# ShunyaoWang/quadruped_locomotion

Measured on NVIDIA B200. Metric: contact-force QPs solved/sec, higher is better.
Workload: dtype f64

## Files before the change

quadruped_locomotion_b200/csrc/qlb_api.cu:

```cuda
#include <cuda_runtime.h>
#include <dlfcn.h>
#include <nccl.h>

#include <cmath>
#include <cstdio>
#include <cstdlib>
#include <cstring>
#include <mutex>
#include <new>

#include "qlb.h"
#include "qlb_aux.cuh"
#include "qlb_gen.cuh"
#include "qlb_qp_dense.cuh"
#include "qlb_records.cuh"
#include "qlb_solve.cuh"
#include "qlb_solve_quad.cuh"
#include "qlb_solve_fused.cuh"
#include "qlb_solve_single.cuh"
#include "qlb_swing.cuh"
#include "qlb_tick.cuh"

using namespace qlb;

#ifndef QLB_PIPE
#define QLB_PIPE 3
#endif
constexpr int kPipe = QLB_PIPE;

struct qlb_context {
  int device = 0;
  int sm_count = 0;
  int blocks_per_sm_quad[2] = {0, 0};
  int blocks_per_sm_first[2] = {0, 0};
  qlb_params params;
  qlb_leg_model legs[QLB_NUM_LEGS];
  DeviceModel* d_model = nullptr;
  DeviceParams* d_params = nullptr;
  DeviceLimbDynamics* d_limb = nullptr;
  DeviceLimbDynamicsT<float>* d_limb_f = nullptr;
  bool have_limb = false;
  DeviceModelT<float>* d_model_f = nullptr;
  DeviceParamsT<float>* d_params_f = nullptr;
  int blocks_per_sm_quad_f[2] = {0, 0};
  int blocks_per_sm_first_f[2] = {0, 0};
  int blocks_per_sm_quad_m[2] = {0, 0};
  int blocks_per_sm_first_m[2] = {0, 0};
  int pipeline = QLB_PIPELINE_FUSED;
  int blocks_per_sm_single[2][2][2] = {};
  std::recursive_mutex mu;
  int fused_bps_cap = 0;
  bool use_tma = true;
  bool f32_pure = false;
  unsigned long long* d_counter = nullptr;
  unsigned* d_list[8] = {};
  size_t list_cap[8] = {};
  uint64_t solve_calls = 0;
  cudaEvent_t slot_done[8] = {};
  int last_slot = 0;
  double* d_stats = nullptr;
  cudaStream_t stream = nullptr;
  cudaStream_t pipe[kPipe] = {};
  double* d_in = nullptr;
  double* d_out = nullptr;
  uint8_t* d_mask = nullptr;
  uint32_t* d_flags = nullptr;
  unsigned char* d_prev = nullptr;
  size_t prev_cap = 0;
  unsigned char* d_qp = nullptr;
  size_t qp_bytes = 0;
  unsigned char* d_rec = nullptr;
  size_t rec_cap = 0;
  size_t cap = 0;
  uint64_t launches = 0;
  char last_error[256] = {0};
};

namespace {

constexpr int kHostInRows = 12 + 7 + 6 + 7 + 6 + 4 + 12;
constexpr int kHostOutRows = 12 + 12 + 6 + 6;
#ifndef QLB_CHUNK_LOG2
#define QLB_CHUNK_LOG2 17
#endif
constexpr size_t kChunk = size_t(1) << QLB_CHUNK_LOG2;

struct DeviceGuard {
  int prev = -1;
  explicit DeviceGuard(int dev) {
// ... 195 lines not shown
}

bool make_mask_map(CUtensorMap* m, const uint8_t* ptr, unsigned long long B, int cols) {
  EncodeTiledFn fn = encode_tiled_fn();
  if (!fn) return false;
  const cuuint64_t gdim[1] = {(cuuint64_t)B};
  const cuuint64_t gstride[1] = {0};
  const cuuint32_t box[1] = {(cuuint32_t)cols};
  const cuuint32_t estr[1] = {1u};
  return fn(m, CU_TENSOR_MAP_DATA_TYPE_UINT8, 1, const_cast<uint8_t*>(ptr), gdim, gstride, box, estr, CU_TENSOR_MAP_INTERLEAVE_NONE,
            CU_TENSOR_MAP_SWIZZLE_NONE, CU_TENSOR_MAP_L2_PROMOTION_NONE, CU_TENSOR_MAP_FLOAT_OOB_FILL_NONE) == CUDA_SUCCESS;
}

template <typename T, typename C, int MODE>
int launch_single(qlb_context* ctx, SolveArgsT<T>& a, cudaStream_t st, const int bps_ipm) {
  using SG = Staging<T, MODE, QLB_SUPER>;
  using FL = FusedLayout<T, C, MODE, QLB_SUPER>;
  const T* src[SG::kNumSeg];
  for (int s = 0; s < SG::kNumSeg; s++) src[s] = SG::source(a, s);
  bool tma = ctx->use_tma && a.B >= 64 && a.B < 0x7fffff00ull && ((a.B * sizeof(T)) % 16 == 0);
  for (int s = 0; s < SG::kNumSeg && tma; s++)
    if (src[s] && !aligned16(src[s])) tma = false;
  FusedMaps maps;
  std::memset(&maps, 0, sizeof maps);
  for (int s = 0; s < SG::kNumSeg && tma; s++)
    if (src[s] && !make_map<T>(&maps.seg[s], src[s], a.B, SG::rows(s))) tma = false;
  if (tma && (SG::kCols < 16 || !aligned16(a.mask) || !make_mask_map(&maps.mask, a.mask, a.B, SG::kCols))) tma = false;
  const unsigned long long ntiles = (a.B + 7) / 8;
  const unsigned long long want = (ntiles + kFusedWarps - 1) / kFusedWarps;
  int bps = ctx->blocks_per_sm_single[sizeof(T) == 4 ? 1 : 0][MODE][tma ? 1 : 0];
  if (ctx->fused_bps_cap > 0 && bps > ctx->fused_bps_cap) bps = ctx->fused_bps_cap;
  const unsigned long long cap = (unsigned long long)ctx->sm_count * bps;
  const unsigned grid = (unsigned)(want < cap ? want : cap);
  if (tma) qlb_single_kernel<T, C, MODE, QLB_SUPER, true><<<grid, kFusedThreads, FL::kTotal, st>>>(a, maps);
  else qlb_single_kernel<T, C, MODE, QLB_SUPER, false><<<grid, kFusedThreads, FL::kTotal, st>>>(a, maps);
  QLB_CUDA(ctx, cudaGetLastError());
  ctx->launches++;
  const unsigned long long capq = (unsigned long long)ctx->sm_count * bps_ipm;
  const unsigned long long wantq = (ntiles + 3) / 4;
  qlb_quad_kernel<T, C, MODE, 2><<<(unsigned)(wantq < capq ? wantq : capq), kQuadThreads, 0, st>>>(a);
  QLB_CUDA(ctx, cudaGetLastError());
  ctx->launches++;
  QLB_CUDA(ctx, cudaEventRecord(ctx->slot_done[ctx->last_slot], st));
  return QLB_OK;
}

template <typename T, typename C, int MODE>
bool prepare_single_kernels(qlb_context* ctx) {
  using FL = FusedLayout<T, C, MODE, QLB_SUPER>;
  int* out = ctx->blocks_per_sm_single[sizeof(T) == 4 ? 1 : 0][MODE];
  if (cudaFuncSetAttribute(qlb_single_kernel<T, C, MODE, QLB_SUPER, false>, cudaFuncAttributeMaxDynamicSharedMemorySize, FL::kTotal) != cudaSuccess ||
      cudaFuncSetAttribute(qlb_single_kernel<T, C, MODE, QLB_SUPER, true>, cudaFuncAttributeMaxDynamicSharedMemorySize, FL::kTotal) != cudaSuccess ||
      cudaFuncSetAttribute(qlb_single_kernel<T, C, MODE, QLB_SUPER, false>, cudaFuncAttributePreferredSharedMemoryCarveout, cudaSharedmemCarveoutMaxShared) != cudaSuccess ||
      cudaFuncSetAttribute(qlb_single_kernel<T, C, MODE, QLB_SUPER, true>, cudaFuncAttributePreferredSharedMemoryCarveout, cudaSharedmemCarveoutMaxShared) != cudaSuccess)
    return false;
  if (cudaOccupancyMaxActiveBlocksPerMultiprocessor(&out[0], qlb_single_kernel<T, C, MODE, QLB_SUPER, false>, kFusedThreads, FL::kTotal) != cudaSuccess ||
      cudaOccupancyMaxActiveBlocksPerMultiprocessor(&out[1], qlb_single_kernel<T, C, MODE, QLB_SUPER, true>, kFusedThreads, FL::kTotal) != cudaSuccess)
    return false;
  return out[0] >= 1 && out[1] >= 1;
}

template <int MODE>
int launch_solve(qlb_context* ctx, SolveArgs& a, cudaStream_t st) {
  const int rc = prepare_slot(ctx, a, st);
  if (rc != QLB_OK) return rc;
  if (ctx->pipeline == QLB_PIPELINE_FUSED) return launch_single<double, double, MODE>(ctx, a, st, ctx->blocks_per_sm_quad[MODE]);
// ... 263 lines not shown
      cudaOccupancyMaxActiveBlocksPerMultiprocessor(&ctx->blocks_per_sm_first_f[0], qlb_quad_first_kernel<float, float, 0>, kQuadThreads, 0) != cudaSuccess ||
      cudaOccupancyMaxActiveBlocksPerMultiprocessor(&ctx->blocks_per_sm_first_f[1], qlb_quad_first_kernel<float, float, 1>, kQuadThreads, 0) != cudaSuccess)
    return fail(QLB_ERR_CUDA);
  if (cudaOccupancyMaxActiveBlocksPerMultiprocessor(&ctx->blocks_per_sm_quad_m[0], qlb_quad_kernel<float, double, 0, 2>, kQuadThreads, 0) != cudaSuccess ||
      cudaOccupancyMaxActiveBlocksPerMultiprocessor(&ctx->blocks_per_sm_quad_m[1], qlb_quad_kernel<float, double, 1, 2>, kQuadThreads, 0) != cudaSuccess ||
      cudaOccupancyMaxActiveBlocksPerMultiprocessor(&ctx->blocks_per_sm_first_m[0], qlb_quad_first_kernel<float, double, 0>, kQuadThreads, 0) != cudaSuccess ||
      cudaOccupancyMaxActiveBlocksPerMultiprocessor(&ctx->blocks_per_sm_first_m[1], qlb_quad_first_kernel<float, double, 1>, kQuadThreads, 0) != cudaSuccess)
    return fail(QLB_ERR_CUDA);
  if (!prepare_single_kernels<double, double, 0>(ctx) || !prepare_single_kernels<double, double, 1>(ctx) ||
      !prepare_single_kernels<float, double, 0>(ctx) || !prepare_single_kernels<float, double, 1>(ctx)) {
    cudaGetLastError();
    return fail(QLB_ERR_CUDA);
  }
  if (const char* e = std::getenv("QLB_FUSED_BPS")) ctx->fused_bps_cap = std::atoi(e);
  if (const char* e = std::getenv("QLB_PIPELINE")) {
    if (!std::strcmp(e, "three_pass")) ctx->pipeline = QLB_PIPELINE_THREE_PASS;

    if (!std::strcmp(e, "fused_notma")) ctx->use_tma = false;
  }
  if (max_batch > 0 && ensure_capacity(ctx, max_batch) != QLB_OK) return fail(QLB_ERR_ALLOC);
  *out = ctx;
  return QLB_OK;
}

int qlb_destroy(qlb_context* ctx) {
  if (!ctx) return QLB_OK;
  DeviceGuard guard(ctx->device);
  if (ctx->stream) { cudaStreamSynchronize(ctx->stream); cudaStreamDestroy(ctx->stream); }
  for (int i = 0; i < kPipe; i++)
    if (ctx->pipe[i]) { cudaStreamSynchronize(ctx->pipe[i]); cudaStreamDestroy(ctx->pipe[i]); }
  cudaFree(ctx->d_model); cudaFree(ctx->d_params); cudaFree(ctx->d_counter); cudaFree(ctx->d_stats);
  cudaFree(ctx->d_model_f); cudaFree(ctx->d_params_f); cudaFree(ctx->d_limb); cudaFree(ctx->d_limb_f);
  cudaFree(ctx->d_in); cudaFree(ctx->d_out); cudaFree(ctx->d_mask); cudaFree(ctx->d_flags); cudaFree(ctx->d_rec); cudaFree(ctx->d_qp); cudaFree(ctx->d_prev);
  for (int i = 0; i < 8; i++) cudaFree(ctx->d_list[i]);
  for (int i = 0; i < 8; i++)
    if (ctx->slot_done[i]) cudaEventDestroy(ctx->slot_done[i]);
  cudaGetLastError();
  delete ctx;
  return QLB_OK;
}

int qlb_set_params(qlb_context* ctx, const qlb_params* params) {
  QLB_GUARD(ctx);
  if (!ctx || !params) return QLB_ERR_INVALID_ARGUMENT;
  if (!params_ok(params)) return QLB_ERR_INVALID_ARGUMENT;
  DeviceGuard guard(ctx->device);
  DeviceParams hp;
  build_device_params(params, &hp);
  QLB_CUDA(ctx, cudaDeviceSynchronize());
  QLB_CUDA(ctx, cudaMemcpy(ctx->d_params, &hp, sizeof hp, cudaMemcpyHostToDevice));
  DeviceParamsT<float> hpf;
  narrow_params(hp, &hpf);
  QLB_CUDA(ctx, cudaMemcpy(ctx->d_params_f, &hpf, sizeof hpf, cudaMemcpyHostToDevice));
  ctx->params = *params;
  return QLB_OK;
}

int qlb_get_params(const qlb_context* ctx, qlb_params* params) {
  if (!ctx || !params) return QLB_ERR_INVALID_ARGUMENT;
  *params = ctx->params;
  return QLB_OK;
}

int qlb_set_f32_core(qlb_context* ctx, int core) {
  QLB_GUARD(ctx);
  if (!ctx) return QLB_ERR_NOT_INITIALISED;
  if (core != QLB_F32_CORE_FP32 && core != QLB_F32_CORE_FP64) return QLB_ERR_INVALID_ARGUMENT;
// ... 1031 lines not shown
```

quadruped_locomotion_b200/csrc/qlb_solve.cuh:

```cuda
#pragma once

#include "qlb_device.cuh"

namespace qlb {

constexpr int kModePolish = 0, kModeIpm = 1, kModeDone = 2;
constexpr int kPolishPasses = 10;
constexpr double kNeighbourhood = 1e-3;

template <typename T>
struct SolveArgsT {
  unsigned long long B;
  const T* q;
  const T* quat;
  const T* wrench;
  const uint8_t* mask;
  const T* mu;
  const T* normals;
  const T* pose;
  const T* twist;
  const T* tpose;
  const T* ttwist;
  T* grf;
  T* tau;
  uint32_t* flags;
  T* netwrench;
  T* wrench_out;
  unsigned long long* counter;
  unsigned long long* counter2;
  unsigned* list;
  unsigned* list_pat;
  unsigned* list_count;
  unsigned long long* counter3;
  unsigned* list2;
  unsigned* list2_count;
  const DeviceModelT<T>* model;
  const DeviceParamsT<T>* params;
  const DeviceParamsT<double>* params64;
};
using SolveArgs = SolveArgsT<double>;

template <typename T>
__device__ __forceinline__ void quat_rel_log(const T* qt, const T* q, T (&v)[3]) {
  const T aw = qt[0], ax = -qt[1], ay = -qt[2], az = -qt[3];
  T w = aw * q[0] - ax * q[1] - ay * q[2] - az * q[3];
  T x = aw * q[1] + ax * q[0] + ay * q[3] - az * q[2];
  T y = aw * q[2] - ax * q[3] + ay * q[0] + az * q[1];
  T z = aw * q[3] + ax * q[2] - ay * q[1] + az * q[0];
  if (w < T(0.0)) { w = -w; x = -x; y = -y; z = -z; }
  const T n = sqrt(x * x + y * y + z * z);
  T k = T(2.0);
  if (n >= T(1e-12)) k = T(2.0) * atan2(n, w) / n;
  v[0] = k * x; v[1] = k * y; v[2] = k * z;
}

}
```

quadruped_locomotion_b200/csrc/qlb_solve_fused.cuh:

```cuda
#pragma once

#include <cuda.h>

#include "qlb_solve_quad.cuh"

namespace qlb {

#ifndef QLB_SUPER
#define QLB_SUPER 2
#endif
#ifndef QLB_DBAS_MAX_ROUNDS
#define QLB_DBAS_MAX_ROUNDS 40
#endif

template <typename real, int MODE, int SUPER>
struct Staging {
  static constexpr int kCols = 8 * SUPER;
  static constexpr int kRow = kCols * (int)sizeof(real);
  __host__ __device__ static constexpr int align(int x) { return (x + 127) & ~127; }
  static constexpr int kNumSeg = (MODE == 1) ? 7 : 5;
  __host__ __device__ static constexpr int rows(int s) {
    return (MODE == 1) ? (s == 0 ? 12 : s == 1 ? 7 : s == 2 ? 6 : s == 3 ? 7 : s == 4 ? 6 : s == 5 ? 4 : 12)
                       : (s == 0 ? 12 : s == 1 ? 4 : s == 2 ? 6 : s == 3 ? 4 : 12);
  }
// ... 31 lines not shown
  asm volatile(
      "{\n"
      ".reg .pred p;\n"
      "mbarrier.try_wait.parity.shared::cta.b64 p, [%1], %2;\n"
      "selp.u32 %0, 1, 0, p;\n"
      "}\n" : "=r"(ok) : "r"(bar), "r"(parity) : "memory");
  return ok != 0u;
}
__device__ __forceinline__ void mbar_wait(uint32_t bar, uint32_t parity) {
  for (unsigned spins = 0; spins < (1u << 24); spins++) {
    const bool ok = mbar_try_wait(bar, parity);
    if (__all_sync(kFull, ok)) break;
  }
}
__device__ __forceinline__ void tma_load_2d(uint32_t dst, const CUtensorMap* map, int c0, int c1, uint32_t bar) {
  asm volatile("cp.async.bulk.tensor.2d.shared::cluster.global.mbarrier::complete_tx::bytes [%0], [%1, {%2, %3}], [%4];"
               ::"r"(dst), "l"(map), "r"(c0), "r"(c1), "r"(bar) : "memory");
}
__device__ __forceinline__ void tma_load_1d(uint32_t dst, const CUtensorMap* map, int c0, uint32_t bar) {
  asm volatile("cp.async.bulk.tensor.1d.shared::cluster.global.mbarrier::complete_tx::bytes [%0], [%1, {%2}], [%3];"
               ::"r"(dst), "l"(map), "r"(c0), "r"(bar) : "memory");
}
__device__ __forceinline__ void cp_async_4(uint32_t dst, const void* src, int valid) {
  asm volatile("cp.async.ca.shared.global [%0], [%1], 4, %2;" ::"r"(dst), "l"(src), "r"(valid) : "memory");
}
__device__ __forceinline__ void cp_async_elem(uint32_t dst, const double* src) {
  asm volatile("cp.async.ca.shared.global [%0], [%1], 8;" ::"r"(dst), "l"(src) : "memory");
}
__device__ __forceinline__ void cp_async_elem(uint32_t dst, const float* src) {
  asm volatile("cp.async.ca.shared.global [%0], [%1], 4;" ::"r"(dst), "l"(src) : "memory");
}
__device__ __forceinline__ void cp_async_commit() { asm volatile("cp.async.commit_group;" ::: "memory"); }
__device__ __forceinline__ void cp_async_wait_all() { asm volatile("cp.async.wait_group 0;" ::: "memory"); }

__device__ __forceinline__ int nth_set_bit(unsigned m, const int j) {
#pragma unroll
  for (int i = 0; i < 7; i++)
    if (i < j) m &= m - 1u;
  return m ? (__ffs(m) - 1) : -1;
}

template <typename real, int MODE, int SUPER, bool TMA>
__device__ __forceinline__ void stage_issue(const SolveArgsT<real>& a, const FusedMaps& maps, const unsigned long long box,
                                            unsigned char* stage, const uint32_t bar, const int lane) {
  using SG = Staging<real, MODE, SUPER>;
  const real* src[SG::kNumSeg];
#pragma unroll
  for (int s = 0; s < SG::kNumSeg; s++) src[s] = SG::source(a, s);
  if (TMA) {
    if (lane == 0) {
      uint32_t bytes = 0;
#pragma unroll
      for (int s = 0; s < SG::kNumSeg; s++)
        if (src[s] != nullptr) bytes += SG::rows(s) * SG::kRow;
      bytes += SG::kCols;
      mbar_expect_tx(bar, bytes);
      const uint32_t dst = smem_u32(stage);
#pragma unroll
      for (int s = 0; s < SG::kNumSeg; s++)
        if (src[s] != nullptr) tma_load_2d(dst + SG::offset(s), &maps.seg[s], (int)(box * (unsigned long long)SG::kCols), 0, bar);
      tma_load_1d(dst + SG::kMaskOff, &maps.mask, (int)(box * (unsigned long long)SG::kCols), bar);
    }
  } else {
    const unsigned long long B = a.B;
    constexpr int kRowsPerPass = 32 / SG::kCols;
    const int col = lane % SG::kCols;
    unsigned long long bx = box * (unsigned long long)SG::kCols + col;
    if (bx >= B) bx = B - 1;
#pragma unroll
    for (int s = 0; s < SG::kNumSeg; s++) {
      if (src[s] == nullptr) continue;
      const uint32_t dst = smem_u32(stage) + SG::offset(s);
#pragma unroll
// ... 195 lines not shown
```

quadruped_locomotion_b200/csrc/qlb_solve_single.cuh:

```cuda
#pragma once

#include "qlb_solve_fused.cuh"

namespace qlb {

#ifndef QLB_FUSED_MIN_CTAS
#define QLB_FUSED_MIN_CTAS 1
#endif
#ifndef QLB_FUSED_MIN_CTAS_F32
#define QLB_FUSED_MIN_CTAS_F32 1
#endif
#ifndef QLB_FUSED_THREADS
#define QLB_FUSED_THREADS 384
#endif
#ifndef QLB_DYNAMIC_PART
#define QLB_DYNAMIC_PART 4
#endif
#ifndef QLB_STASH_CAP
#define QLB_STASH_CAP 22
#endif
#ifndef QLB_ROUND_LOW
#define QLB_ROUND_LOW 8
#endif
constexpr int kFusedThreads = QLB_FUSED_THREADS;
constexpr int kFusedWarps = kFusedThreads / 32;
template <typename real> constexpr int fused_min_ctas() { return sizeof(real) == 4 ? QLB_FUSED_MIN_CTAS_F32 : QLB_FUSED_MIN_CTAS; }
template <typename real> constexpr int fused_smem_budget() { return (228 / fused_min_ctas<real>() - 1) * 1024; }

constexpr int kStashLane = 16;
constexpr int kSlFoot = 6, kSlMu = 9, kSlY = 10, kSlU = 13;
template <typename real, typename creal, int CAP>
struct StashLayout {
  static constexpr int kQ = 4 * CAP;
  static constexpr int kLaneBytes = kStashLane * kQ * (int)sizeof(creal);
  static constexpr int kJBytes = 12 * kQ * (int)sizeof(real);
  static constexpr int kBBytes = 6 * CAP * (int)sizeof(creal);
  static constexpr int kHBytes = 4 * CAP * 4;
  static constexpr int kBytes = ((kLaneBytes + kJBytes + kBBytes + kHBytes) + 15) & ~15;
};

template <typename real, typename creal, int MODE, int SUPER>
struct FusedLayout {
  static constexpr int kCtlWords = 8;
  static constexpr int kBarBytes = (kFusedWarps * 8 + 63) & ~63;
  static constexpr int kFixed = ((((int)sizeof(DeviceParamsT<real>) + 15) & ~15) + (((int)sizeof(CoreConst<creal>) + 15) & ~15) + kBarBytes +
                                 kFusedWarps * kCtlWords * 4 + 127) & ~127;
  static constexpr int kStatic = (int)sizeof(DeviceModelT<double>) + 128;
  static constexpr int kStage = Staging<real, MODE, SUPER>::kBytes;
  static constexpr int stash_bytes(int c) {
    return ((kStashLane * 4 * c * (int)sizeof(creal) + 12 * 4 * c * (int)sizeof(real) + 6 * c * (int)sizeof(creal) + 16 * c) + 15) & ~15;
  }
  static constexpr int warp_bytes(int c) { return (kStage + stash_bytes(c) + 127) & ~127; }
  static constexpr int cap_for(int c) { return (kStatic + kFixed + kFusedWarps * warp_bytes(c) <= fused_smem_budget<real>() || c <= 8) ? c : cap_for(c - 1); }
  static constexpr int kCap = cap_for(QLB_STASH_CAP);
  static_assert(kCap >= 10, "stash too small");
  static_assert(stash_bytes(kCap) == StashLayout<real, creal, kCap>::kBytes, "layout mismatch");
  static constexpr int kWarpBytes = warp_bytes(kCap);
  static constexpr int kTotal = kFixed + kFusedWarps * kWarpBytes;
  static_assert(kStatic + kTotal <= fused_smem_budget<real>(), "shared memory budget");
};

template <typename real, typename creal, int CAP>
struct WarpStash {
  creal* sl;
  real* sj;
  creal* sb;
  uint32_t* sh;
  __device__ WarpStash(unsigned char* base) {
    using SL = StashLayout<real, creal, CAP>;
    sl = reinterpret_cast<creal*>(base);
    sj = reinterpret_cast<real*>(base + SL::kLaneBytes);
    sb = reinterpret_cast<creal*>(base + SL::kLaneBytes + SL::kJBytes);
    sh = reinterpret_cast<uint32_t*>(base + SL::kLaneBytes + SL::kJBytes + SL::kBBytes);
  }
};


template <typename real, typename creal, int CAP>
__device__ __forceinline__ void stash_load(const WarpStash<real, creal, CAP>& ws, const int slot, const int leg, RoundState<creal>& q) {
  constexpr int Q = 4 * CAP;
  const int e = 4 * slot + leg;
  const uint32_t w1 = ws.sh[CAP + slot];
  q.idx = ws.sh[slot];
  q.gscale = __uint_as_float(ws.sh[2 * CAP + slot]);
  q.mask = w1 & 0xFu;
  q.alive = (w1 >> leg) & 1u;
  q.rounds = (int)(w1 >> 24);
  const unsigned pat = (w1 >> (4 + 5 * leg)) & 31u;
  q.a0 = (int)(pat & 1u);
  q.sg1 = ((pat >> 1) & 3u) == 1u ? -1 : (((pat >> 1) & 3u) == 2u ? 1 : 0);
  q.sg2 = ((pat >> 3) & 3u) == 1u ? -1 : (((pat >> 3) & 3u) == 2u ? 1 : 0);
  creal foot[3];
#pragma unroll
  for (int c = 0; c < 3; c++) {
    q.At[0][c] = ws.sl[c * Q + e];
    q.At[1][c] = ws.sl[(3 + c) * Q + e];
    foot[c] = ws.sl[(kSlFoot + c) * Q + e];
  }
  {
    creal t2[3];
    t2[0] = q.At[0][1] * q.At[1][2] - q.At[0][2] * q.At[1][1];
    t2[1] = q.At[0][2] * q.At[1][0] - q.At[0][0] * q.At[1][2];
    t2[2] = q.At[0][0] * q.At[1][1] - q.At[0][1] * q.At[1][0];
    const creal rn = q.alive ? fast_rsqrt(t2[0] * t2[0] + t2[1] * t2[1] + t2[2] * t2[2]) : creal(0.0);
#pragma unroll
    for (int c = 0; c < 3; c++) q.At[2][c] = t2[c] * rn;
  }
  q.mu = ws.sl[kSlMu * Q + e];
#pragma unroll
  for (int c = 0; c < 3; c++) { q.y[c] = ws.sl[(kSlY + c) * Q + e]; q.u[c] = ws.sl[(kSlU + c) * Q + e]; }
#pragma unroll
  for (int c = 0; c < 3; c++) {
    q.At[c][3] = foot[1] * q.At[c][2] - foot[2] * q.At[c][1];
    q.At[c][4] = foot[2] * q.At[c][0] - foot[0] * q.At[c][2];
    q.At[c][5] = foot[0] * q.At[c][1] - foot[1] * q.At[c][0];
  }
}

__device__ __forceinline__ unsigned pattern_bits(const int a0, const int sg1, const int sg2) {
  return (a0 != 0 ? 1u : 0u) | (sg1 == -1 ? 2u : (sg1 == 1 ? 4u : 0u)) | (sg2 == -1 ? 8u : (sg2 == 1 ? 16u : 0u));
}

template <typename real, typename creal, int CAP>
__device__ __forceinline__ void stash_save(const WarpStash<real, creal, CAP>& ws, const int slot, const int leg, const RoundState<creal>& q,
                                           const bool doit) {
  constexpr int Q = 4 * CAP;
  const unsigned pat = quad_or(pattern_bits(q.a0, q.sg1, q.sg2) << (5 * leg));
  if (doit) {
    const int e = 4 * slot + leg;
#pragma unroll
    for (int c = 0; c < 3; c++) { ws.sl[(kSlY + c) * Q + e] = q.y[c]; ws.sl[(kSlU + c) * Q + e] = q.u[c]; }
    if (leg == 0) ws.sh[CAP + slot] = q.mask | (pat << 4) | ((unsigned)q.rounds << 24);
  }
}

template <typename real, typename creal, int CAP>
__device__ __forceinline__ void round_phase(const SolveArgsT<real>& a, const CoreConst<creal>& cc, const WarpStash<real, creal, CAP>& ws,
                                            unsigned& occ, const bool final, const int run_min, const int lane, const int leg,
                                            const int quad) {
  constexpr int Q = 4 * CAP;
  unsigned unassigned = occ;
  RoundState<creal> q;
#pragma unroll
  for (int c = 0; c < 3; c++) {
#pragma unroll
    for (int r = 0; r < 6; r++) q.At[c][r] = creal(0.0);
    q.y[c] = creal(0.0); q.u[c] = creal(0.0);
  }
  q.mu = creal(0.0); q.a0 = 0; q.sg1 = 0; q.sg2 = 0; q.gscale = 1.f; q.mask = 0u; q.alive = false; q.rounds = 0; q.idx = 0u;
  int slot = nth_set_bit(unassigned, quad);
  bool active = slot >= 0;
  {
    const int ntake = min(8, __popc(unassigned));
#pragma unroll 1
    for (int i = 0; i < ntake; i++) unassigned &= unassigned - 1u;
  }
  bool fresh = active;
#pragma unroll 1
  for (;;) {
    if (fresh) stash_load(ws, slot, leg, q);
    fresh = false;
    bool done, fail;
    const int bslot = active ? slot : 0;
    dbas_round<creal>(q, ws.sb + bslot, CAP, cc, leg, active, done, fail);
    const bool leave = active && (done || fail);
    if (__any_sync(kFull, leave)) {
      LegSetup<creal> L;
#pragma unroll
      for (int c = 0; c < 3; c++) {
#pragma unroll
        for (int r = 0; r < 6; r++) L.At[c][r] = q.At[c][r];
      }
      L.alive = q.alive; L.mask = q.mask;
      const int oslot = active ? slot : 0;
      quad_output<real, creal, real>(a, L, q.y, q.a0, q.sg1, q.sg2, 0, q.rounds, (unsigned long long)q.idx, active && done, leg,
                               ws.sj + 4 * oslot + leg, Q);
      const unsigned fm = __ballot_sync(kFull, active && fail && leg == 0);
      if (fm != 0u) {
        unsigned base = 0;
        if (lane == 0) base = atomicAdd(a.list2_count, __popc(fm));
        base = __shfl_sync(kFull, base, 0);
        if (active && fail && leg == 0) a.list2[base + __popc(fm & ((1u << lane) - 1u))] = q.idx;
      }
      const unsigned freed = __reduce_or_sync(kFull, leave ? (1u << slot) : 0u);
      occ &= ~freed;
      const unsigned wm = __ballot_sync(kFull, leave && leg == 0);
      const int rank = __popc(wm & ((1u << (lane & ~3)) - 1u));
      __syncwarp();
      if (leave) {
        slot = nth_set_bit(unassigned, rank);
        active = slot >= 0;
        fresh = active;
      }
      {
        const int ntake = min(__popc(wm), __popc(unassigned));
#pragma unroll 1
        for (int i = 0; i < ntake; i++) unassigned &= unassigned - 1u;
      }
    }
    const int nact = __popc(__ballot_sync(kFull, active && leg == 0));
    if (nact == 0) break;
    if (!final && nact + __popc(unassigned) < run_min) {
      stash_save(ws, active ? slot : 0, leg, q, active && !fresh);
      break;
    }
  }
  __syncwarp();
}

template <typename real, typename creal, int MODE, int SUPER, bool TMA>
__global__ void __launch_bounds__(kFusedThreads, fused_min_ctas<real>())
qlb_single_kernel(const SolveArgsT<real> a, const __grid_constant__ FusedMaps maps) {
  using FL = FusedLayout<real, creal, MODE, SUPER>;
  constexpr int CAP = FL::kCap;
  constexpr int Q = 4 * CAP;
  constexpr int kRunMin = CAP - 7;
  constexpr int kRunLow = QLB_ROUND_LOW < kRunMin ? QLB_ROUND_LOW : kRunMin;
  constexpr int kCols = 8 * SUPER;
  extern __shared__ __align__(128) unsigned char smem[];
  DeviceParamsT<real>& prm = *reinterpret_cast<DeviceParamsT<real>*>(smem);
  CoreConst<creal>& cc = *reinterpret_cast<CoreConst<creal>*>(smem + ((sizeof(DeviceParamsT<real>) + 15) & ~15));
  static_assert(((sizeof(DeviceParamsT<real>) + 15) & ~15) + sizeof(CoreConst<creal>) + FL::kBarBytes + kFusedWarps * FL::kCtlWords * 4 <= FL::kFixed, "fixed part");
  unsigned long long* bars = reinterpret_cast<unsigned long long*>(smem + FL::kFixed - FL::kBarBytes);
  volatile unsigned* ctl = reinterpret_cast<volatile unsigned*>(smem + FL::kFixed - FL::kBarBytes - kFusedWarps * FL::kCtlWords * 4) +
                           (threadIdx.x >> 5) * FL::kCtlWords;
  const int warp = threadIdx.x >> 5, lane = threadIdx.x & 31;
  const int leg = lane & 3, quad = lane >> 2;
  unsigned char* wbase = smem + FL::kFixed + warp * FL::kWarpBytes;
  unsigned char* stage = wbase;
  const WarpStash<real, creal, CAP> ws(wbase + FL::kStage);
  const uint32_t bar = smem_u32(&bars[warp]);
  {
    const uint32_t* src = reinterpret_cast<const uint32_t*>(a.params);
    uint32_t* dst = reinterpret_cast<uint32_t*>(&prm);
    for (int i = threadIdx.x; i < (int)(sizeof(DeviceParamsT<real>) / 4); i += blockDim.x) dst[i] = src[i];
    cc.load(a.params64);
    load_model_to_smem(a.model);
    if (TMA && lane == 0) {
      mbar_init(bar, 1);
      asm volatile("fence.mbarrier_init.release.cluster;" ::: "memory");
      asm volatile("fence.proxy.async.shared::cta;" ::: "memory");
    }
  }
  __syncthreads();
  const unsigned nbox = (unsigned)((a.B + kCols - 1) / kCols);
  unsigned occ = 0u;

  const unsigned nwarps = gridDim.x * kFusedWarps;
  const unsigned gwarp = blockIdx.x * kFusedWarps + warp;
  const unsigned share = (nbox - nbox / QLB_DYNAMIC_PART) / nwarps;
  const unsigned dyn_base = share * nwarps;
  if (lane == 0) { ctl[0] = share; ctl[1] = dyn_base; ctl[2] = 0u; ctl[3] = nbox; ctl[4] = (unsigned)a.B; ctl[5] = 0u; ctl[6] = 0u; }
  __syncwarp();
  auto claim_raw = [&](const bool doit) -> unsigned {
    unsigned b = 0;
    if (lane == 0 && doit) b = atomicAdd(reinterpret_cast<unsigned*>(a.counter), 1u);
    return b;
  };
  unsigned pending_claim = claim_raw(share <= 1);
  unsigned cur;
  {
    cur = __shfl_sync(kFull, share > 0 ? gwarp : dyn_base + pending_claim, 0);
    if (share == 0) pending_claim = claim_raw(true);
  }
  if (cur < nbox) stage_issue<real, MODE, SUPER, TMA>(a, maps, cur, stage, bar, lane);
  if (lane == 0) ctl[5] = (cur < nbox) ? 0x200u : 0u;
  __syncwarp();
  unsigned nxt = 0;
#pragma unroll 1
  for (;;) {
    const unsigned cw = __shfl_sync(kFull, ctl[5], 0);
    const bool have = (cw & 0x200u) != 0u;
    if (have) {
      const int sub = (int)(cw & 0xffu);
      const unsigned cw_wait = (sub == 0 && TMA) ? (cw ^ 0x100u) : cw;
      if (sub + 1 < SUPER && lane == 0) ctl[5] = cw_wait + 1u;
      if (sub == 0) {
        if (TMA) mbar_wait(bar, (cw >> 8) & 1u);
        else { cp_async_wait_all(); __syncwarp(); }
      }
      const int col = sub * 8 + quad;
      const unsigned s0 = cur * kCols + col, Bu = ctl[4];
      const bool valid = s0 < Bu;
      const unsigned bq = valid ? s0 : (Bu - 1u);
      RawIn<real, MODE> in;
      stage_read<real, MODE, SUPER>(a, stage, prm.mu_default, leg, col, bq, in);
      if (!valid) in.mask = 0u;
      if (sub == SUPER - 1) {
        __syncwarp();
        const unsigned taken = __shfl_sync(kFull, ctl[2], 0) + 1u, shr = __shfl_sync(kFull, ctl[0], 0);
        if (lane == 0) ctl[2] = taken;
        nxt = __shfl_sync(kFull, taken < shr ? blockIdx.x * kFusedWarps + warp + taken * (gridDim.x * kFusedWarps) : ctl[1] + pending_claim, 0);
        pending_claim = claim_raw(taken + 1 >= shr);
        const bool more = nxt < __shfl_sync(kFull, ctl[3], 0);
        if (lane == 0) ctl[5] = (cw_wait & 0x100u) | (more ? 0x200u : 0u);
        if (more) stage_issue<real, MODE, SUPER, TMA>(a, maps, nxt, stage, bar, lane);
      }
      const int slot = nth_set_bit(~occ & ((1u << CAP) - 1u), quad);
      LegSetup<creal> L;
      quad_setup<real, MODE, creal>(a, prm, in, bq, valid, true, leg, L, ws.sj + 4 * slot + leg, Q);
      int status;
      creal y[3], t[6];
      bool hard;
      unsigned pat;
      quad_first_solve<real, creal>(L, cc.sinv, cc.winv, cc.fmin, leg, y, t, status, hard, pat);
      hard = hard && valid;
      creal net[6];
#pragma unroll
      for (int r = 0; r < 6; r++) net[r] = fma(-cc.sinv[r], t[r], L.b[r]);
      quad_output<real, creal, real>(a, L, y, 0, 0, 0, status, 0, bq, valid, leg, ws.sj + 4 * slot + leg, Q, net);
      if (hard) {
        const int e = 4 * slot + leg;
#pragma unroll
        for (int c = 0; c < 3; c++) {
#pragma unroll
          for (int k = 0; k < 2; k++) ws.sl[(3 * k + c) * Q + e] = L.At[k][c];
          ws.sl[(kSlFoot + c) * Q + e] = L.foot[c];
          ws.sl[(kSlY + c) * Q + e] = y[c];
          ws.sl[(kSlU + c) * Q + e] = creal(0.0);
        }
        ws.sl[kSlMu * Q + e] = L.mu;
        ws.sb[leg * CAP + slot] = sel4(leg, L.b[0], L.b[1], L.b[2], L.b[3]);
        if (leg < 2) ws.sb[(4 + leg) * CAP + slot] = (leg & 1) ? L.b[5] : L.b[4];
        if (leg == 0) {
          ws.sh[slot] = (unsigned)bq;
          ws.sh[CAP + slot] = L.mask | (pat << 4);
          ws.sh[2 * CAP + slot] = __float_as_uint(L.gscale);
        }
      }
      occ |= __reduce_or_sync(kFull, hard ? (1u << slot) : 0u);
      __syncwarp();
      if (sub + 1 == SUPER) cur = nxt;
    }
    const int pending = __popc(occ);
    if (have ? (pending >= kRunMin) : (pending > 0)) round_phase<real, creal, CAP>(a, cc, ws, occ, !have, kRunLow, lane, leg, quad);
    if (!have) break;
  }
}

}
```

Measured before the change: 2.273 billion.

## Replace per-warp stash with block-shared pool of hard QP states

Replaces each warp's private stash of hard (unresolved) contact QPs with a block-wide shared-memory pool. The pool is managed by a free list, a pending list and per-block global-memory overflow buffers. Tile phases fill the pool until it is nearly full, then all warps synchronise and drain it together in a round phase that claims work from a shared counter. This is meant to improve load balance and keep more lanes busy in the iterative DBAS rounds, at the cost of block-wide __syncthreads barriers, shared-memory atomics, and overflow traffic through global memory.

```diff
diff --git a/quadruped_locomotion_b200/csrc/qlb_api.cu b/quadruped_locomotion_b200/csrc/qlb_api.cu
--- a/quadruped_locomotion_b200/csrc/qlb_api.cu
+++ b/quadruped_locomotion_b200/csrc/qlb_api.cu
@@ -55,6 +55,8 @@
   unsigned long long* d_counter = nullptr;
   unsigned* d_list[8] = {};
   size_t list_cap[8] = {};
+  unsigned char* d_overflow[8] = {};
+  size_t overflow_bytes[8] = {};
   uint64_t solve_calls = 0;
   cudaEvent_t slot_done[8] = {};
   int last_slot = 0;
@@ -316,6 +318,17 @@
   if (ctx->fused_bps_cap > 0 && bps > ctx->fused_bps_cap) bps = ctx->fused_bps_cap;
   const unsigned long long cap = (unsigned long long)ctx->sm_count * bps;
   const unsigned grid = (unsigned)(want < cap ? want : cap);
+  const int slot = ctx->last_slot;
+  const size_t ov_bytes = (size_t)grid * FL::kOvBytes;
+  if (ctx->overflow_bytes[slot] < ov_bytes) {
+    QLB_CUDA(ctx, cudaDeviceSynchronize());
+    cudaFree(ctx->d_overflow[slot]);
+    ctx->d_overflow[slot] = nullptr;
+    ctx->overflow_bytes[slot] = 0;
+    if (cudaMalloc(&ctx->d_overflow[slot], ov_bytes) != cudaSuccess) { cudaGetLastError(); return QLB_ERR_ALLOC; }
+    ctx->overflow_bytes[slot] = ov_bytes;
+  }
+  a.overflow = ctx->d_overflow[slot];
   if (tma) qlb_single_kernel<T, C, MODE, QLB_SUPER, true><<<grid, kFusedThreads, FL::kTotal, st>>>(a, maps);
   else qlb_single_kernel<T, C, MODE, QLB_SUPER, false><<<grid, kFusedThreads, FL::kTotal, st>>>(a, maps);
   QLB_CUDA(ctx, cudaGetLastError());
@@ -645,7 +658,7 @@
   cudaFree(ctx->d_model); cudaFree(ctx->d_params); cudaFree(ctx->d_counter); cudaFree(ctx->d_stats);
   cudaFree(ctx->d_model_f); cudaFree(ctx->d_params_f); cudaFree(ctx->d_limb); cudaFree(ctx->d_limb_f);
   cudaFree(ctx->d_in); cudaFree(ctx->d_out); cudaFree(ctx->d_mask); cudaFree(ctx->d_flags); cudaFree(ctx->d_rec); cudaFree(ctx->d_qp); cudaFree(ctx->d_prev);
-  for (int i = 0; i < 8; i++) cudaFree(ctx->d_list[i]);
+  for (int i = 0; i < 8; i++) { cudaFree(ctx->d_list[i]); cudaFree(ctx->d_overflow[i]); }
   for (int i = 0; i < 8; i++)
     if (ctx->slot_done[i]) cudaEventDestroy(ctx->slot_done[i]);
   cudaGetLastError();
diff --git a/quadruped_locomotion_b200/csrc/qlb_pool.cuh b/quadruped_locomotion_b200/csrc/qlb_pool.cuh
--- /dev/null
+++ b/quadruped_locomotion_b200/csrc/qlb_pool.cuh
@@ -0,0 +1,44 @@
+#pragma once
+
+#ifndef __CUDACC__
+#ifndef __host__
+#define __host__
+#endif
+#ifndef __device__
+#define __device__
+#endif
+#endif
+
+namespace qlb {
+
+struct PoolCtl {
+  unsigned top;
+  unsigned ntake;
+  unsigned npend0;
+  unsigned head;
+  unsigned npush;
+  unsigned npark;
+  unsigned long long ov;
+};
+
+enum { kClaimPool = 0, kClaimOverflow = 1, kClaimNone = 2 };
+enum { kRoundDone = 0, kRoundPark = 1, kRoundRun = 2 };
+
+template <int P, int TILE_LOW, int ROUND_LOW>
+struct PoolRules {
+  static_assert(ROUND_LOW >= 1 && TILE_LOW >= 1 && ROUND_LOW + TILE_LOW <= P,
+                "a round phase that stops must leave TILE_LOW slots free, or the next tile phase could not start");
+  __host__ __device__ static bool tile_go(const unsigned top, const unsigned ntake) { return ntake + TILE_LOW <= top; }
+  __host__ __device__ static unsigned placed(const unsigned top, const unsigned ntake) { return ntake < top ? ntake : top; }
+  __host__ __device__ static unsigned npend(const unsigned npend0, const unsigned top, const unsigned ntake) { return npend0 + placed(top, ntake); }
+  __host__ __device__ static unsigned nov(const unsigned top, const unsigned ntake) { return ntake > top ? ntake - top : 0u; }
+  __host__ __device__ static unsigned base(const unsigned top, const unsigned ntake) { return top - placed(top, ntake); }
+  __host__ __device__ static int claim(const unsigned c, const unsigned npend, const unsigned nov, const bool holds) {
+    return c < npend ? kClaimPool : (c < npend + nov && holds) ? kClaimOverflow : kClaimNone;
+  }
+  __host__ __device__ static int round_next(const int nact, const bool final) {
+    return nact == 0 ? kRoundDone : (!final && nact < ROUND_LOW) ? kRoundPark : kRoundRun;
+  }
+};
+
+}
diff --git a/quadruped_locomotion_b200/csrc/qlb_solve.cuh b/quadruped_locomotion_b200/csrc/qlb_solve.cuh
--- a/quadruped_locomotion_b200/csrc/qlb_solve.cuh
+++ b/quadruped_locomotion_b200/csrc/qlb_solve.cuh
@@ -37,6 +37,7 @@
   const DeviceModelT<T>* model;
   const DeviceParamsT<T>* params;
   const DeviceParamsT<double>* params64;
+  unsigned char* overflow;
 };
 using SolveArgs = SolveArgsT<double>;
 
diff --git a/quadruped_locomotion_b200/csrc/qlb_solve_fused.cuh b/quadruped_locomotion_b200/csrc/qlb_solve_fused.cuh
--- a/quadruped_locomotion_b200/csrc/qlb_solve_fused.cuh
+++ b/quadruped_locomotion_b200/csrc/qlb_solve_fused.cuh
@@ -87,13 +87,6 @@
 }
 __device__ __forceinline__ void cp_async_commit() { asm volatile("cp.async.commit_group;" ::: "memory"); }
 __device__ __forceinline__ void cp_async_wait_all() { asm volatile("cp.async.wait_group 0;" ::: "memory"); }
-
-__device__ __forceinline__ int nth_set_bit(unsigned m, const int j) {
-#pragma unroll
-  for (int i = 0; i < 7; i++)
-    if (i < j) m &= m - 1u;
-  return m ? (__ffs(m) - 1) : -1;
-}
 
 template <typename real, int MODE, int SUPER, bool TMA>
 __device__ __forceinline__ void stage_issue(const SolveArgsT<real>& a, const FusedMaps& maps, const unsigned long long box,
diff --git a/quadruped_locomotion_b200/csrc/qlb_solve_single.cuh b/quadruped_locomotion_b200/csrc/qlb_solve_single.cuh
--- a/quadruped_locomotion_b200/csrc/qlb_solve_single.cuh
+++ b/quadruped_locomotion_b200/csrc/qlb_solve_single.cuh
@@ -1,6 +1,7 @@
 #pragma once
 
 #include "qlb_solve_fused.cuh"
+#include "qlb_pool.cuh"
 
 namespace qlb {
 
@@ -16,14 +17,15 @@
 #ifndef QLB_DYNAMIC_PART
 #define QLB_DYNAMIC_PART 4
 #endif
-#ifndef QLB_STASH_CAP
-#define QLB_STASH_CAP 22
+#ifndef QLB_POOL_TILE_LOW
+#define QLB_POOL_TILE_LOW 24
 #endif
 #ifndef QLB_ROUND_LOW
-#define QLB_ROUND_LOW 8
+#define QLB_ROUND_LOW 84
 #endif
 constexpr int kFusedThreads = QLB_FUSED_THREADS;
 constexpr int kFusedWarps = kFusedThreads / 32;
+constexpr int kOvCap = 8 * kFusedWarps;
 template <typename real> constexpr int fused_min_ctas() { return sizeof(real) == 4 ? QLB_FUSED_MIN_CTAS_F32 : QLB_FUSED_MIN_CTAS; }
 template <typename real> constexpr int fused_smem_budget() { return (228 / fused_min_ctas<real>() - 1) * 1024; }
 
@@ -44,29 +46,33 @@
   static constexpr int kCtlWords = 8;
   static constexpr int kBarBytes = (kFusedWarps * 8 + 63) & ~63;
   static constexpr int kFixed = ((((int)sizeof(DeviceParamsT<real>) + 15) & ~15) + (((int)sizeof(CoreConst<creal>) + 15) & ~15) + kBarBytes +
-                                 kFusedWarps * kCtlWords * 4 + 127) & ~127;
+                                 kFusedWarps * kCtlWords * 4 + (int)sizeof(PoolCtl) + 127) & ~127;
   static constexpr int kStatic = (int)sizeof(DeviceModelT<double>) + 128;
   static constexpr int kStage = Staging<real, MODE, SUPER>::kBytes;
-  static constexpr int stash_bytes(int c) {
-    return ((kStashLane * 4 * c * (int)sizeof(creal) + 12 * 4 * c * (int)sizeof(real) + 6 * c * (int)sizeof(creal) + 16 * c) + 15) & ~15;
-  }
-  static constexpr int warp_bytes(int c) { return (kStage + stash_bytes(c) + 127) & ~127; }
-  static constexpr int cap_for(int c) { return (kStatic + kFixed + kFusedWarps * warp_bytes(c) <= fused_smem_budget<real>() || c <= 8) ? c : cap_for(c - 1); }
-  static constexpr int kCap = cap_for(QLB_STASH_CAP);
-  static_assert(kCap >= 10, "stash too small");
-  static_assert(stash_bytes(kCap) == StashLayout<real, creal, kCap>::kBytes, "layout mismatch");
-  static constexpr int kWarpBytes = warp_bytes(kCap);
-  static constexpr int kTotal = kFixed + kFusedWarps * kWarpBytes;
+  static constexpr int kScratch = 12 * 32 * (int)sizeof(real);
+  static constexpr int kWarpBytes = (kStage + kScratch + 127) & ~127;
+  static constexpr int kEntry = kStashLane * 4 * (int)sizeof(creal) + 12 * 4 * (int)sizeof(real) + 6 * (int)sizeof(creal) + 16;
+  static constexpr int kPoolRoom = fused_smem_budget<real>() - kStatic - kFixed - kFusedWarps * kWarpBytes - 32;
+  static constexpr int kPool = kPoolRoom / (kEntry + 4);
+  static_assert(kPool >= kOvCap && kPool < 65536, "the pool must hold a state for every quad (qlb_pool.cuh)");
+  static constexpr int kPoolBytes = StashLayout<real, creal, kPool>::kBytes;
+  static constexpr int kListBytes = (2 * kPool * 2 + 15) & ~15;
+  static constexpr int kPoolOff = kFixed + kFusedWarps * kWarpBytes;
+  static constexpr int kPcOff = kFixed - kBarBytes - kFusedWarps * kCtlWords * 4 - (int)sizeof(PoolCtl);
+  static constexpr int kTotal = kPoolOff + kPoolBytes + kListBytes;
   static_assert(kStatic + kTotal <= fused_smem_budget<real>(), "shared memory budget");
+  static constexpr int kOvBytes = StashLayout<real, creal, kOvCap>::kBytes;
+  static constexpr int kRoundLow = QLB_ROUND_LOW < kPool - QLB_POOL_TILE_LOW ? QLB_ROUND_LOW : kPool - QLB_POOL_TILE_LOW;
+  using Rules = PoolRules<kPool, QLB_POOL_TILE_LOW, kRoundLow>;
 };
 
 template <typename real, typename creal, int CAP>
-struct WarpStash {
+struct Stash {
   creal* sl;
   real* sj;
   creal* sb;
   uint32_t* sh;
-  __device__ WarpStash(unsigned char* base) {
+  __device__ Stash(unsigned char* base) {
     using SL = StashLayout<real, creal, CAP>;
     sl = reinterpret_cast<creal*>(base);
     sj = reinterpret_cast<real*>(base + SL::kLaneBytes);
@@ -77,7 +83,7 @@
 
 
 template <typename real, typename creal, int CAP>
-__device__ __forceinline__ void stash_load(const WarpStash<real, creal, CAP>& ws, const int slot, const int leg, RoundState<creal>& q) {
+__device__ __forceinline__ void stash_load(const Stash<real, creal, CAP>& ws, const int slot, const int leg, RoundState<creal>& q) {
   constexpr int Q = 4 * CAP;
   const int e = 4 * slot + leg;
   const uint32_t w1 = ws.sh[CAP + slot];
@@ -117,12 +123,50 @@
   }
 }
 
+template <typename real, typename creal, int CAP>
+__device__ __forceinline__ void stash_put(const Stash<real, creal, CAP>& ws, const int slot, const int leg, const LegSetup<creal>& L,
+                                          const creal (&y)[3], const unsigned pat, const unsigned idx, const real* jw) {
+  constexpr int Q = 4 * CAP;
+  const int e = 4 * slot + leg;
+#pragma unroll
+  for (int c = 0; c < 3; c++) {
+#pragma unroll
+    for (int k = 0; k < 2; k++) ws.sl[(3 * k + c) * Q + e] = L.At[k][c];
+    ws.sl[(kSlFoot + c) * Q + e] = L.foot[c];
+    ws.sl[(kSlY + c) * Q + e] = y[c];
+    ws.sl[(kSlU + c) * Q + e] = creal(0.0);
+  }
+  ws.sl[kSlMu * Q + e] = L.mu;
+#pragma unroll
+  for (int k = 0; k < 12; k++) ws.sj[k * Q + e] = jw[k * 32];
+  ws.sb[leg * CAP + slot] = sel4(leg, L.b[0], L.b[1], L.b[2], L.b[3]);
+  if (leg < 2) ws.sb[(4 + leg) * CAP + slot] = (leg & 1) ? L.b[5] : L.b[4];
+  if (leg == 0) {
+    ws.sh[slot] = idx;
+    ws.sh[CAP + slot] = L.mask | (pat << 4);
+    ws.sh[2 * CAP + slot] = __float_as_uint(L.gscale);
+  }
+}
+
+template <typename real, typename creal, int P, int OV>
+__device__ __forceinline__ void stash_move(const Stash<real, creal, OV>& os, const int o, const Stash<real, creal, P>& ps, const int slot,
+                                           const int leg) {
+  const int e = 4 * slot + leg, f = 4 * o + leg;
+#pragma unroll 1
+  for (int k = 0; k < kStashLane; k++) ps.sl[k * 4 * P + e] = os.sl[k * 4 * OV + f];
+#pragma unroll 1
+  for (int k = 0; k < 12; k++) ps.sj[k * 4 * P + e] = os.sj[k * 4 * OV + f];
+  ps.sb[leg * P + slot] = os.sb[leg * OV + o];
+  if (leg < 2) ps.sb[(4 + leg) * P + slot] = os.sb[(4 + leg) * OV + o];
+  if (leg < 3) ps.sh[leg * P + slot] = os.sh[leg * OV + o];
+}
+
 __device__ __forceinline__ unsigned pattern_bits(const int a0, const int sg1, const int sg2) {
   return (a0 != 0 ? 1u : 0u) | (sg1 == -1 ? 2u : (sg1 == 1 ? 4u : 0u)) | (sg2 == -1 ? 8u : (sg2 == 1 ? 16u : 0u));
 }
 
 template <typename real, typename creal, int CAP>
-__device__ __forceinline__ void stash_save(const WarpStash<real, creal, CAP>& ws, const int slot, const int leg, const RoundState<creal>& q,
+__device__ __forceinline__ void stash_save(const Stash<real, creal, CAP>& ws, const int slot, const int leg, const RoundState<creal>& q,
                                            const bool doit) {
   constexpr int Q = 4 * CAP;
   const unsigned pat = quad_or(pattern_bits(q.a0, q.sg1, q.sg2) << (5 * leg));
@@ -134,12 +178,21 @@
   }
 }
 
-template <typename real, typename creal, int CAP>
-__device__ __forceinline__ void round_phase(const SolveArgsT<real>& a, const CoreConst<creal>& cc, const WarpStash<real, creal, CAP>& ws,
-                                            unsigned& occ, const bool final, const int run_min, const int lane, const int leg,
-                                            const int quad) {
-  constexpr int Q = 4 * CAP;
-  unsigned unassigned = occ;
+__device__ __forceinline__ unsigned quad_atomic_rank(unsigned* ctr, const unsigned m, const int lane) {
+  unsigned c0 = 0;
+  if (lane == 0) c0 = atomicAdd(ctr, (unsigned)__popc(m));
+  return __shfl_sync(kFull, c0, 0) + (unsigned)__popc(m & ((1u << (lane & ~3)) - 1u));
+}
+
+template <typename FL, typename real, typename creal, int P>
+__device__ __forceinline__ void round_phase(const SolveArgsT<real>& a, const CoreConst<creal>& cc, const bool final, const int lane,
+                                            const int leg) {
+  using R = typename FL::Rules;
+  extern __shared__ __align__(128) unsigned char smem[];
+  const Stash<real, creal, P> ps(smem + FL::kPoolOff);
+  uint16_t* const freel = reinterpret_cast<uint16_t*>(smem + FL::kPoolOff + FL::kPoolBytes);
+  uint16_t* const pend = freel + P;
+  PoolCtl& pc = *reinterpret_cast<PoolCtl*>(smem + FL::kPcOff);
   RoundState<creal> q;
 #pragma unroll
   for (int c = 0; c < 3; c++) {
@@ -148,61 +201,69 @@
     q.y[c] = creal(0.0); q.u[c] = creal(0.0);
   }
   q.mu = creal(0.0); q.a0 = 0; q.sg1 = 0; q.sg2 = 0; q.gscale = 1.f; q.mask = 0u; q.alive = false; q.rounds = 0; q.idx = 0u;
-  int slot = nth_set_bit(unassigned, quad);
-  bool active = slot >= 0;
-  {
-    const int ntake = min(8, __popc(unassigned));
-#pragma unroll 1
-    for (int i = 0; i < ntake; i++) unassigned &= unassigned - 1u;
-  }
-  bool fresh = active;
+  int slot = -1;
+  bool active = false;
 #pragma unroll 1
   for (;;) {
-    if (fresh) stash_load(ws, slot, leg, q);
-    fresh = false;
-    bool done, fail;
-    const int bslot = active ? slot : 0;
-    dbas_round<creal>(q, ws.sb + bslot, CAP, cc, leg, active, done, fail);
-    const bool leave = active && (done || fail);
-    if (__any_sync(kFull, leave)) {
-      LegSetup<creal> L;
-#pragma unroll
-      for (int c = 0; c < 3; c++) {
-#pragma unroll
-        for (int r = 0; r < 6; r++) L.At[c][r] = q.At[c][r];
-      }
-      L.alive = q.alive; L.mask = q.mask;
-      const int oslot = active ? slot : 0;
-      quad_output<real, creal, real>(a, L, q.y, q.a0, q.sg1, q.sg2, 0, q.rounds, (unsigned long long)q.idx, active && done, leg,
-                               ws.sj + 4 * oslot + leg, Q);
-      const unsigned fm = __ballot_sync(kFull, active && fail && leg == 0);
-      if (fm != 0u) {
-        unsigned base = 0;
-        if (lane == 0) base = atomicAdd(a.list2_count, __popc(fm));
-        base = __shfl_sync(kFull, base, 0);
-        if (active && fail && leg == 0) a.list2[base + __popc(fm & ((1u << lane) - 1u))] = q.idx;
-      }
-      const unsigned freed = __reduce_or_sync(kFull, leave ? (1u << slot) : 0u);
-      occ &= ~freed;
-      const unsigned wm = __ballot_sync(kFull, leave && leg == 0);
-      const int rank = __popc(wm & ((1u << (lane & ~3)) - 1u));
+    const unsigned im = __ballot_sync(kFull, !active && leg == 0);
+    if (im != 0u) {
+      const unsigned c = quad_atomic_rank(&pc.head, im, lane);
+      const volatile PoolCtl& vc = pc;
+      const unsigned top = vc.top, ntake = vc.ntake;
+      const unsigned npend = R::npend(vc.npend0, top, ntake), nov = R::nov(top, ntake);
+      const int kind = active ? kClaimNone : R::claim(c, npend, nov, slot >= 0);
+      const bool take = !active && kind != kClaimNone;
+      const bool release = !active && slot >= 0 && kind != kClaimOverflow;
+      const unsigned rm = __ballot_sync(kFull, release && leg == 0);
+      if (rm != 0u) {
+        const unsigned p = quad_atomic_rank(&pc.npush, rm, lane);
+        if (release && leg == 0) freel[R::base(top, ntake) + p] = (uint16_t)slot;
+      }
+      if (kind == kClaimPool && !active) slot = pend[c];
+      else if (kind == kClaimOverflow && !active)
+        stash_move<real, creal, P, kOvCap>(Stash<real, creal, kOvCap>(reinterpret_cast<unsigned char*>(vc.ov)), (int)(c - npend), ps, slot, leg);
+      else if (release) slot = -1;
+      if (take) stash_load(ps, slot, leg, q);
+      active = active || take;
       __syncwarp();
-      if (leave) {
-        slot = nth_set_bit(unassigned, rank);
-        active = slot >= 0;
-        fresh = active;
-      }
-      {
-        const int ntake = min(__popc(wm), __popc(unassigned));
-#pragma unroll 1
-        for (int i = 0; i < ntake; i++) unassigned &= unassigned - 1u;
-      }
-    }
-    const int nact = __popc(__ballot_sync(kFull, active && leg == 0));
-    if (nact == 0) break;
-    if (!final && nact + __popc(unassigned) < run_min) {
-      stash_save(ws, active ? slot : 0, leg, q, active && !fresh);
+    }
+    const int nact = __shfl_sync(kFull, __syncthreads_count(active && leg == 0), 0);
+    const int next = R::round_next(nact, final);
+    if (next == kRoundDone) break;
+    if (next == kRoundPark) {
+      stash_save(ps, slot, leg, q, active);
+      const unsigned km = __ballot_sync(kFull, active && leg == 0);
+      if (km != 0u) {
+        const unsigned k = quad_atomic_rank(&pc.npark, km, lane);
+        if (active && leg == 0) pend[k] = (uint16_t)slot;
+      }
       break;
+    }
+    if (__any_sync(kFull, active)) {
+      bool done, fail;
+      const int bslot = active ? slot : 0;
+      dbas_round<creal>(q, ps.sb + bslot, P, cc, leg, active, done, fail);
+      const bool leave = active && (done || fail);
+      if (__any_sync(kFull, leave)) {
+        LegSetup<creal> L;
+#pragma unroll
+        for (int c = 0; c < 3; c++) {
+#pragma unroll
+          for (int r = 0; r < 6; r++) L.At[c][r] = q.At[c][r];
+        }
+        L.alive = q.alive; L.mask = q.mask;
+        const unsigned idx = ps.sh[bslot];
+        quad_output<real, creal, real>(a, L, q.y, q.a0, q.sg1, q.sg2, 0, q.rounds, (unsigned long long)idx, active && done, leg,
+                                 ps.sj + 4 * bslot + leg, 4 * P);
+        const unsigned fm = __ballot_sync(kFull, active && fail && leg == 0);
+        if (fm != 0u) {
+          unsigned base = 0;
+          if (lane == 0) base = atomicAdd(a.list2_count, __popc(fm));
+          base = __shfl_sync(kFull, base, 0);
+          if (active && fail && leg == 0) a.list2[base + __popc(fm & ((1u << lane) - 1u))] = idx;
+        }
+        active = active && !leave;
+      }
     }
   }
   __syncwarp();
@@ -212,23 +273,25 @@
 __global__ void __launch_bounds__(kFusedThreads, fused_min_ctas<real>())
 qlb_single_kernel(const SolveArgsT<real> a, const __grid_constant__ FusedMaps maps) {
   using FL = FusedLayout<real, creal, MODE, SUPER>;
-  constexpr int CAP = FL::kCap;
-  constexpr int Q = 4 * CAP;
-  constexpr int kRunMin = CAP - 7;
-  constexpr int kRunLow = QLB_ROUND_LOW < kRunMin ? QLB_ROUND_LOW : kRunMin;
+  using R = typename FL::Rules;
+  constexpr int P = FL::kPool;
   constexpr int kCols = 8 * SUPER;
   extern __shared__ __align__(128) unsigned char smem[];
   DeviceParamsT<real>& prm = *reinterpret_cast<DeviceParamsT<real>*>(smem);
   CoreConst<creal>& cc = *reinterpret_cast<CoreConst<creal>*>(smem + ((sizeof(DeviceParamsT<real>) + 15) & ~15));
-  static_assert(((sizeof(DeviceParamsT<real>) + 15) & ~15) + sizeof(CoreConst<creal>) + FL::kBarBytes + kFusedWarps * FL::kCtlWords * 4 <= FL::kFixed, "fixed part");
+  static_assert(((sizeof(DeviceParamsT<real>) + 15) & ~15) + sizeof(CoreConst<creal>) + FL::kBarBytes + kFusedWarps * FL::kCtlWords * 4 +
+                sizeof(PoolCtl) <= FL::kFixed, "fixed part");
   unsigned long long* bars = reinterpret_cast<unsigned long long*>(smem + FL::kFixed - FL::kBarBytes);
   volatile unsigned* ctl = reinterpret_cast<volatile unsigned*>(smem + FL::kFixed - FL::kBarBytes - kFusedWarps * FL::kCtlWords * 4) +
                            (threadIdx.x >> 5) * FL::kCtlWords;
+  PoolCtl& pc = *reinterpret_cast<PoolCtl*>(smem + FL::kPcOff);
+  const volatile PoolCtl& vpc = pc;
   const int warp = threadIdx.x >> 5, lane = threadIdx.x & 31;
   const int leg = lane & 3, quad = lane >> 2;
-  unsigned char* wbase = smem + FL::kFixed + warp * FL::kWarpBytes;
-  unsigned char* stage = wbase;
-  const WarpStash<real, creal, CAP> ws(wbase + FL::kStage);
+  unsigned char* stage = smem + FL::kFixed + warp * FL::kWarpBytes;
+  const Stash<real, creal, P> ps(smem + FL::kPoolOff);
+  uint16_t* freel = reinterpret_cast<uint16_t*>(smem + FL::kPoolOff + FL::kPoolBytes);
+  uint16_t* pend = freel + P;
   const uint32_t bar = smem_u32(&bars[warp]);
   {
     const uint32_t* src = reinterpret_cast<const uint32_t*>(a.params);
@@ -236,6 +299,10 @@
     for (int i = threadIdx.x; i < (int)(sizeof(DeviceParamsT<real>) / 4); i += blockDim.x) dst[i] = src[i];
     cc.load(a.params64);
     load_model_to_smem(a.model);
+    for (int i = threadIdx.x; i < P; i += blockDim.x) freel[i] = (uint16_t)i;
+    if (threadIdx.x == 0) { pc.top = P; pc.ntake = 0u; pc.npend0 = 0u; pc.head = 0u; pc.npush = 0u; pc.npark = 0u;
+      pc.ov = reinterpret_cast<unsigned long long>(a.overflow + (size_t)blockIdx.x * FL::kOvBytes);
+    }
     if (TMA && lane == 0) {
       mbar_init(bar, 1);
       asm volatile("fence.mbarrier_init.release.cluster;" ::: "memory");
@@ -244,7 +311,6 @@
   }
   __syncthreads();
   const unsigned nbox = (unsigned)((a.B + kCols - 1) / kCols);
-  unsigned occ = 0u;
 
   const unsigned nwarps = gridDim.x * kFusedWarps;
   const unsigned gwarp = blockIdx.x * kFusedWarps + warp;
@@ -266,12 +332,12 @@
   if (cur < nbox) stage_issue<real, MODE, SUPER, TMA>(a, maps, cur, stage, bar, lane);
   if (lane == 0) ctl[5] = (cur < nbox) ? 0x200u : 0u;
   __syncwarp();
-  unsigned nxt = 0;
 #pragma unroll 1
   for (;;) {
     const unsigned cw = __shfl_sync(kFull, ctl[5], 0);
     const bool have = (cw & 0x200u) != 0u;
-    if (have) {
+    const bool go = __shfl_sync(kFull, (have && R::tile_go(vpc.top, vpc.ntake)) ? 1u : 0u, 0) != 0u;
+    if (go) {
       const int sub = (int)(cw & 0xffu);
       const unsigned cw_wait = (sub == 0 && TMA) ? (cw ^ 0x100u) : cw;
       if (sub + 1 < SUPER && lane == 0) ctl[5] = cw_wait + 1u;
@@ -286,6 +352,7 @@
       RawIn<real, MODE> in;
       stage_read<real, MODE, SUPER>(a, stage, prm.mu_default, leg, col, bq, in);
       if (!valid) in.mask = 0u;
+      unsigned nxt = cur;
       if (sub == SUPER - 1) {
         __syncwarp();
         const unsigned taken = __shfl_sync(kFull, ctl[2], 0) + 1u, shr = __shfl_sync(kFull, ctl[0], 0);
@@ -296,9 +363,9 @@
         if (lane == 0) ctl[5] = (cw_wait & 0x100u) | (more ? 0x200u : 0u);
         if (more) stage_issue<real, MODE, SUPER, TMA>(a, maps, nxt, stage, bar, lane);
       }
-      const int slot = nth_set_bit(~occ & ((1u << CAP) - 1u), quad);
+      real* const jw = reinterpret_cast<real*>(stage + FL::kStage) + 4 * quad + leg;
       LegSetup<creal> L;
-      quad_setup<real, MODE, creal>(a, prm, in, bq, valid, true, leg, L, ws.sj + 4 * slot + leg, Q);
+      quad_setup<real, MODE, creal>(a, prm, in, bq, valid, true, leg, L, jw, 32);
       int status;
       creal y[3], t[6];
       bool hard;
@@ -308,34 +375,39 @@
       creal net[6];
 #pragma unroll
       for (int r = 0; r < 6; r++) net[r] = fma(-cc.sinv[r], t[r], L.b[r]);
-      quad_output<real, creal, real>(a, L, y, 0, 0, 0, status, 0, bq, valid, leg, ws.sj + 4 * slot + leg, Q, net);
-      if (hard) {
-        const int e = 4 * slot + leg;
-#pragma unroll
-        for (int c = 0; c < 3; c++) {
-#pragma unroll
-          for (int k = 0; k < 2; k++) ws.sl[(3 * k + c) * Q + e] = L.At[k][c];
-          ws.sl[(kSlFoot + c) * Q + e] = L.foot[c];
-          ws.sl[(kSlY + c) * Q + e] = y[c];
-          ws.sl[(kSlU + c) * Q + e] = creal(0.0);
+      quad_output<real, creal, real>(a, L, y, 0, 0, 0, status, 0, bq, valid, leg, jw, 32, net);
+      const unsigned hm = __ballot_sync(kFull, hard && leg == 0);
+      if (hm != 0u) {
+        const unsigned c = quad_atomic_rank(&pc.ntake, hm, lane);
+        if (hard) {
+          const unsigned top = vpc.top;
+          if (c < top) {
+            const int slot = freel[top - 1u - c];
+            if (leg == 0) pend[vpc.npend0 + c] = (uint16_t)slot;
+            stash_put(ps, slot, leg, L, y, pat, bq, jw);
+          } else {
+            stash_put(Stash<real, creal, kOvCap>(reinterpret_cast<unsigned char*>(vpc.ov)), (int)(c - top), leg, L, y, pat, bq, jw);
+          }
         }
-        ws.sl[kSlMu * Q + e] = L.mu;
-        ws.sb[leg * CAP + slot] = sel4(leg, L.b[0], L.b[1], L.b[2], L.b[3]);
-        if (leg < 2) ws.sb[(4 + leg) * CAP + slot] = (leg & 1) ? L.b[5] : L.b[4];
-        if (leg == 0) {
-          ws.sh[slot] = (unsigned)bq;
-          ws.sh[CAP + slot] = L.mask | (pat << 4);
-          ws.sh[2 * CAP + slot] = __float_as_uint(L.gscale);
-        }
-      }
-      occ |= __reduce_or_sync(kFull, hard ? (1u << slot) : 0u);
+      }
       __syncwarp();
       if (sub + 1 == SUPER) cur = nxt;
-    }
-    const int pending = __popc(occ);
-    if (have ? (pending >= kRunMin) : (pending > 0)) round_phase<real, creal, CAP>(a, cc, ws, occ, !have, kRunLow, lane, leg, quad);
-    if (!have) break;
-  }
-}
-
-}
+      continue;
+    }
+    if (lane == 0) { ctl[6] = pending_claim; ctl[7] = cur; }
+    const bool any = __shfl_sync(kFull, __syncthreads_or(have ? 1 : 0), 0) != 0;
+    if (!any && __shfl_sync(kFull, R::npend(vpc.npend0, vpc.top, vpc.ntake) + R::nov(vpc.top, vpc.ntake), 0) == 0u) break;
+    round_phase<FL, real, creal, P>(a, cc, !any, lane, leg);
+    __syncthreads();
+    if (threadIdx.x == 0) {
+      pc.top = R::base(vpc.top, vpc.ntake) + pc.npush;
+      pc.npend0 = pc.npark;
+      pc.ntake = 0u; pc.head = 0u; pc.npush = 0u; pc.npark = 0u;
+    }
+    __syncthreads();
+    pending_claim = ctl[6];
+    cur = __shfl_sync(kFull, ctl[7], 0);
+  }
+}
+
+}
```

Result: slower. 767.7 million, median of 6 (-66.2%).
